# rebots-online/InstantIR

Measured on AMD Instinct MI355X. Metric: denoising steps/sec at 1024x1024 (InstantIR step: previewer UNet + LCM + Aggregator + UNet, CFG), higher is better.
Workload: dtype f16 (fp32 accumulate); 1 GPU; BASELINE configs[1]: 1024x1024, batch 1/GPU, cfg 7.0 (2 rows), 30-step DDIM timetable, preview_start 0, full SDXL+TA-IP UNet x2 + Aggregator per step; images_per_gpu=1, weight_elements=4422072388, graph=True, finite=True, world=1

## Files before the change

instantir_amd/csrc/gemm8.hip:

```cpp
#include "common.h"
#include "gemm_geo.h"
#include "../../include/instantir_hip.h"

namespace {

using iir::Geo;
constexpr int BK = 64;
constexpr int PF_TOUCHES = 2;

template <int BN, bool F8 = false>
__global__ __launch_bounds__(512, 2) void gemm8_kernel(const Geo g) {
    using E = f16;
    using E4 = f16x4;
    using E8 = f16x8;
    constexpr int BM = 256, NT = 512;
    constexpr int WM = 128, WN = BN / 4, MI = WM / 16, NI = WN / 16;
    constexpr int A_BYTES = BM * 128, B_BYTES = BN * 128, STAGE = A_BYTES + B_BYTES, RING_BYTES = 2 * STAGE;
    constexpr int A_PIECES = BM / 64, B_PIECES = BN / 64;
    static_assert(BN % 64 == 0 && NI * 16 == WN && B_PIECES <= MI - 1, "tile shape");
    extern __shared__ __attribute__((aligned(16))) char smem[];
    float2* rowstat = (float2*)(smem + RING_BYTES + 2048);

    const int tid = threadIdx.x, lane = tid & 63;
    const int wave = __builtin_amdgcn_readfirstlane(tid >> 6);
    const int wm = wave >> 2, wn = wave & 3;

    int tm, tn;
    if (!iir::tile_of_block(g, tm, tn)) return;
    const int m0 = tm * BM, n0 = tn * BN;

    const int srow = lane >> 3, schunk = (lane & 7) ^ srow;
    const unsigned a_voff = (unsigned)(srow * (int)g.lda * 2 + schunk * 16);
    const unsigned b_voff = (unsigned)(srow * g.K * 2 + schunk * 16);
    const char* a_base = (const char*)g.A + (long)(m0 + wave * 8) * g.lda * 2;
    const char* b_base = (const char*)g.W + (long)(n0 + wave * 8) * g.K * 2;
    const long a_pstride = 64L * g.lda * 2, b_pstride = 64L * g.K * 2;
    auto stage_a = [&](int t, int buf) {
#pragma unroll
        for (int q = 0; q < A_PIECES; ++q)
            glds16(a_base + q * a_pstride + t * 128 + a_voff, smem + buf * STAGE + (q * 8 + wave) * 1024);
    };
    auto stage_b1 = [&](int t, int buf, int q) {
        glds16(b_base + q * b_pstride + t * 128 + b_voff, smem + buf * STAGE + A_BYTES + (q * 8 + wave) * 1024);
    };

    const int frow = lane & 15, fq = lane >> 4;
    int a_off[2], b_off[2];
#pragma unroll
    for (int s = 0; s < 2; ++s) {
        const int phys = (s * 4 + fq) ^ (frow & 7);
        a_off[s] = (wm * WM + frow) * 128 + phys * 16;
        b_off[s] = A_BYTES + (wn * WN + frow) * 128 + phys * 16;
    }

    f32x4 acc[MI][NI];
#pragma unroll
    for (int i = 0; i < MI; ++i)
#pragma unroll
        for (int j = 0; j < NI; ++j) acc[i][j] = (f32x4){0.f, 0.f, 0.f, 0.f};

    const int nk = g.K / BK;
    stage_a(0, 0);
#pragma unroll
    for (int q = 0; q < B_PIECES; ++q) stage_b1(0, 0, q);
    if (nk > 1) {
#pragma unroll
        for (int q = 0; q < B_PIECES; ++q) stage_b1(1, 1, q);
    }

    if (g.ln_in && tid < BM) rowstat[tid] = iir::ln_row_stat(g, min(m0 + tid, g.M - 1));

    E8 bfr[2][NI], a0[2], a1[2];
    auto read_b = [&](const char* st) {
#pragma unroll
        for (int s = 0; s < 2; ++s)
#pragma unroll
            for (int j = 0; j < NI; ++j) bfr[s][j] = *(const E8*)(st + b_off[s] + j * 2048);
    };
    auto read_a = [&](const char* st, int i, E8 (&a)[2]) {
#pragma unroll
        for (int s = 0; s < 2; ++s) a[s] = *(const E8*)(st + a_off[s] + i * 2048);
    };

    if (nk > 1) asm volatile("s_waitcnt vmcnt(%0)\n\ts_barrier" ::"n"(B_PIECES) : "memory");
    else asm volatile("s_waitcnt vmcnt(0)\n\ts_barrier" ::: "memory");

    int cur = 0;
    for (int t = 0; t < nk; ++t) {
        const char* st = smem + cur * STAGE;
        read_b(st);
        read_a(st, 0, a0);
        const bool more_a = t + 1 < nk, more_b = t + 2 < nk;
        if (more_a) stage_a(t + 1, cur ^ 1);
        auto piece = [&](int i) { if (i >= 1 && i <= B_PIECES && more_b) stage_b1(t + 2, cur, i - 1); };
#pragma unroll
        for (int i = 0; i < MI; ++i) {
            E8(&ac)[2] = (i & 1) ? a1 : a0;
            E8(&an)[2] = (i & 1) ? a0 : a1;
            if (i + 1 < MI) read_a(st, i + 1, an);
            piece(i);
            __builtin_amdgcn_s_setprio(1);
#pragma unroll
            for (int s = 0; s < 2; ++s)
#pragma unroll
                for (int j = 0; j < NI; ++j) {
                    if constexpr (F8) acc[i][j] = iir::mfma16_f8x2(bfr[s][j], ac[s], acc[i][j]);
                    else acc[i][j] = __builtin_amdgcn_mfma_f32_16x16x32_f16(bfr[s][j], ac[s], acc[i][j], 0, 0, 0);
                }
            __builtin_amdgcn_s_setprio(0);
            if (i == 0) asm volatile("s_waitcnt lgkmcnt(0)\n\ts_barrier" ::: "memory");
        }
        if (more_b) asm volatile("s_waitcnt vmcnt(%0) lgkmcnt(0)\n\ts_barrier" ::"n"(B_PIECES) : "memory");
        else asm volatile("s_waitcnt vmcnt(0) lgkmcnt(0)\n\ts_barrier" ::: "memory");
        cur ^= 1;
    }

    const bool paired = g.epi != IIR_EPI_PLAIN;
    const int cs = (paired ? BN : 2 * BN) + 32;
    constexpr int CHUNK_ROWS = 64, STAGE_STRIDE = CHUNK_ROWS * (2 * BN + 32);
    f32x4 c1v[NI], scv[F8 ? NI : 1];
    E4 c0v[NI];
#pragma unroll
    for (int j = 0; j < NI; ++j) {
        const int nc = n0 + wn * WN + j * 16 + fq * 4;
        c1v[j] = g.ln_in ? *(const f32x4*)(g.ln_colsum + nc) : (f32x4){0.f, 0.f, 0.f, 0.f};
        if constexpr (F8) scv[j] = *(const f32x4*)(g.wscale + nc) * g.a_scale;
        if (g.bias) c0v[j] = *(const E4*)(g.bias + nc);
        else for (int t = 0; t < 4; ++t) c0v[j][t] = (E)0.f;
    }
    const int cpr = paired ? BN / 16 : BN / 8;
    const int no_tile = paired ? n0 / 2 : n0;
    const bool use_res = g.res && !paired;
    const int total = CHUNK_ROWS * cpr;
    iir::touch_next_weights<NT, PF_TOUCHES>(g, tid, smem + RING_BYTES + wave * 256);
#pragma unroll
    for (int c = 0; c < MI / 2; ++c) {
        char* ct = smem + (c & 1) * STAGE_STRIDE;
#pragma unroll
        for (int ii = 0; ii < 2; ++ii) {
            const int i = 2 * c + ii;
            const int lr = wm * WM + i * 16 + frow;
            const float2 rs = g.ln_in ? rowstat[lr] : make_float2(1.f, 0.f);
            char* rowp = ct + (wm * 32 + ii * 16 + frow) * cs;
#pragma unroll
            for (int j = 0; j < NI; ++j) {
                float a[4];
#pragma unroll
                for (int t = 0; t < 4; ++t) a[t] = iir::epi_affine(F8 ? acc[i][j][t] * scv[F8 ? j : 0][t] : acc[i][j][t], rs, c1v[j][t], (float)c0v[j][t]);
                if (!paired) {
                    iir::epi_act(g.act, a);
                    E4 o;
                    for (int t = 0; t < 4; ++t) o[t] = (E)a[t];
                    *(E4*)(rowp + (wn * WN + j * 16 + fq * 4) * 2) = o;
                } else {
                    int col;
                    const f16x2 o2 = iir::geglu_pair<E>(a, fq, col);
                    *(f16x2*)(rowp + ((wn * WN + j * 16) / 2 + col) * 2) = o2;
                }
            }
        }
        asm volatile("s_waitcnt lgkmcnt(0)\n\ts_barrier" ::: "memory");
        if (g.Ct && n0 >= g.tr_from) {
#pragma unroll 1
            for (int p = tid; p < BN * (CHUNK_ROWS / 8); p += NT) {
                const int col = p >> 3, gq = p & 7;
                const long m = m0 + (gq >> 2) * WM + c * 32 + (gq & 3) * 8;
                E8 o;
#pragma unroll
                for (int t = 0; t < 8; ++t) o[t] = (E)((float)*(const E*)(ct + (gq * 8 + t) * cs + col * 2) * g.out_scale);
                *(E8*)(g.Ct + (long)(n0 + col - g.tr_from) * g.ldct + m) = o;
            }
            continue;
        }
#pragma unroll 1
        for (int p = tid; p < total; p += NT) {
            const int s = p / cpr, cc = p - s * cpr;
            const long m = m0 + (s >> 5) * WM + c * 32 + (s & 31);
            const E8 v = *(const E8*)(ct + s * cs + cc * 16);
            E8 o;
            if (use_res) {
                const E8 rr = *(const E8*)(g.res + m * g.ldr + no_tile + cc * 8);
                for (int t = 0; t < 8; ++t) o[t] = (E)(((float)v[t] + (float)rr[t]) * g.out_scale);
            } else {
                for (int t = 0; t < 8; ++t) o[t] = (E)((float)v[t] * g.out_scale);
            }
            if (g.c_fp8) *(long*)((char*)g.C + m * g.ldc + no_tile + cc * 8) = iir_fp8x8(o);
            else iir::store16(g.C, (m * g.ldc + no_tile + cc * 8) * 2, o, g.st_wt != 0);
        }
    }
    asm volatile("s_waitcnt vmcnt(0)" ::: "memory");
}

template <int BN, bool F8 = false>
int launch8(const Geo& g0, hipStream_t stream) {
    constexpr int BM = 256;
    Geo g = g0;
    iir::xcd_partition(g, BM, BN, HUGE_VAL);
    const size_t lds = 2 * (BM * 128 + BN * 128) + 2048 + BM * 8;
    static unsigned long long lds_set = 0;
    if (!iir_ensure_dynamic_lds((const void*)gemm8_kernel<BN, F8>, lds, lds_set)) return IIR_ELAUNCH;
    iir_launch(gemm8_kernel<BN, F8>, dim3(8 * g.rm * g.rn), dim3(512), lds, stream, g);
    return iir_launch_status();
}

}

namespace iir {

bool gemm8_covers(const Geo& g, int bn) {
    if (bn != 320 && bn != 256) return false;
    if (g.dtype != IIR_DT_F16 || g.c_f32 || g.ln_out || g.gn_out || (g.wscale && !g.f8) || g.rowbias || g.xa_on) return false;
    if (g.f8 && (g.ln_in || g.Ct || bn != 320)) return false;
    if (g.c_fp8 && (g.ldc % 8 || (uintptr_t)g.C % 8)) return false;
    if (g.Ct && (g.epi != IIR_EPI_PLAIN || g.res || g.tr_from % bn || !g.ct_vec)) return false;
    if (g.epi != IIR_EPI_PLAIN && g.epi != IIR_EPI_GEGLU) return false;
    if (g.M % 256 || g.N % bn || g.K % 64 || g.K < 128) return false;
    if ((!g.c_vec && !g.c_fp8) || (g.res && g.epi == IIR_EPI_PLAIN && !g.r_vec)) return false;
    if (g.lda % 8 || ((uintptr_t)g.A % 16) || ((uintptr_t)g.W % 16)) return false;
    if (g.bias && ((uintptr_t)g.bias % 8)) return false;
    if (g.ln_in && g.ln_parts > 8) return false;
    if ((long)g.lda * 2 * 7 + 128 >= (1L << 31) || (long)g.K * 2 * 7 + 128 >= (1L << 31)) return false;
    return true;
}

int gemm8_launch(const Geo& g, int bn, hipStream_t stream) {
    if (!gemm8_covers(g, bn)) return IIR_EINVAL;
    if (g.f8) return launch8<320, true>(g, stream);
    return bn == 320 ? launch8<320>(g, stream) : launch8<256>(g, stream);
}

}
```

instantir_amd/csrc/gemm_conv.hip:

```cpp
#include "common.h"
#include "gemm_geo.h"
#include "../../include/instantir_hip.h"
#include <stdlib.h>
#include <type_traits>

namespace {

using iir::Geo;

constexpr int BK = 64;
#define IIR_PIN() __builtin_amdgcn_sched_barrier(0)
constexpr int PF_TOUCHES = 4;

constexpr int gn_par(int bm, bool lw) { return lw && bm == 128 ? 2 : 1; }
constexpr int ring_bytes(int bm, int bn, int st, bool w8) { return st * (bm * 128 + (w8 ? bn * 64 : bn * 128)); }
constexpr int scratch_bytes(int waves_m, bool lw) { return 256 * waves_m * 2 * (lw ? 2 : 1); }
constexpr int lds_bytes(int bm, int bn, int st, int waves_m, bool w8, bool lw) { return ring_bytes(bm, bn, st, w8) + scratch_bytes(waves_m, lw) + bm * 8; }
constexpr int lnp_off(int bm, int bn) { return (bm * (2 * bn + 32) + 15) / 16 * 16; }
constexpr bool ln_out_fits(int bm, int bn, int st, bool w8) { return lnp_off(bm, bn) + bm * (bn / 8) * 8 <= ring_bytes(bm, bn, st, w8); }
constexpr bool gn_out_fits(int bm, int bn, int st, int nt, bool lw, bool w8 = false) {
    const int gnt = nt / gn_par(bm, lw);
    return bm % 64 == 0 && bn <= gnt && (long)lnp_off(bm, bn) + (long)gn_par(bm, lw) * (gnt / (bn / 8)) * bn * 8 <= ring_bytes(bm, bn, st, w8);
}

// ... 734 lines not shown
    if (g.gn_out) {
        constexpr bool fits = gn_out_fits(BM, BN, ST, NT, LW, W8);
        if (!fits || g.epi != IIR_EPI_PLAIN || g.c_f32 || g.Ct || g.ln_out || g.M % BM || g.N % BN || !g.c_vec || (g.res && !g.r_vec) ||
            (CONV && (g.y_img_rows | g.res_img_rows)))
            return IIR_EINVAL;
    }
    if (g.ln_out) {
        constexpr bool fits = ln_out_fits(BM, BN, ST, W8);
        if (!fits || CONV || g.epi != IIR_EPI_PLAIN || g.c_f32 || g.Ct || g.M % BM || g.N % BN || !g.c_vec || (g.res && !g.r_vec))
            return IIR_EINVAL;
    }
    iir::xcd_partition(g, BM, BN, 3.0 * 1048576.);
    const dim3 grid(8 * g.rm * g.rn), block(NT);
    const auto kern = gemm_kernel<E, BM, BN, ST, CONV, WAVES_M, W8, LW, F8>;
    static unsigned long long lds_set = 0;
    if (!iir_ensure_dynamic_lds((const void*)kern, lds, lds_set)) return IIR_ELAUNCH;
    iir_launch(kern, grid, block, lds, stream, g);
    return iir_launch_status();
}

template <int BM, int BN, int ST, int WAVES_M = 2, bool LW = false>
int launch(const Geo& g, bool conv, hipStream_t stream) {
    constexpr bool T5_3 = BM == 64 && BN == 160 && ST == 3 && WAVES_M == 2;
    constexpr bool FP8_TILE = T5_3 || (ST == 2 && WAVES_M == 2 && !LW);
    if (g.f8 || g.wscale) {
        if (conv || g.dtype != IIR_DT_F16) return IIR_EINVAL;
        if constexpr (FP8_TILE) {
            if (g.f8) return launch_k<f16, BM, BN, ST, false, WAVES_M, false, LW, true>(g, stream);
            if constexpr (!LW) return launch_k<f16, BM, BN, ST, false, WAVES_M, true>(g, stream);
        }
        return IIR_EINVAL;
    }
    if (g.dtype == IIR_DT_BF16) {
        if constexpr (ST == 2 && WAVES_M == 2 && !LW)
            return conv ? launch_k<bf16, BM, BN, ST, true>(g, stream) : launch_k<bf16, BM, BN, ST, false>(g, stream);
        return IIR_EINVAL;
    }
    if (!conv) return launch_k<f16, BM, BN, ST, false, WAVES_M, false, LW>(g, stream);
    if constexpr (!LW || ST == 3) return launch_k<f16, BM, BN, ST, true, WAVES_M, false, LW>(g, stream);
    return IIR_EINVAL;
}

struct TileShape { int bm, bn; };
constexpr TileShape kTiles[] = {{0, 0}, {128, 128}, {128, 64}, {64, 64}, {128, 160}, {64, 160}, {256, 128}};
constexpr int N_TILES = sizeof(kTiles) / sizeof(kTiles[0]) - 1;

constexpr int ONE_PER_CU_MIN_K = 1280;

int pick_tile(int M, int N, bool paired, int K = 0) {
    if (K >= ONE_PER_CU_MIN_K && (long)((M + 63) / 64) * ((N + 159) / 160) <= 256) return 5;
    long best = -1;
    int pick = 1;
    for (int t = 1; t <= 5; ++t) {
        const long blocks = (long)((M + kTiles[t].bm - 1) / kTiles[t].bm) * ((N + kTiles[t].bn - 1) / kTiles[t].bn);
        const long cost = ((blocks + 511) / 512) * 2 * (kTiles[t].bm + kTiles[t].bn);
        if (best < 0 || cost < best || (cost == best && kTiles[t].bm * kTiles[t].bn > kTiles[pick].bm * kTiles[pick].bn)) {
            best = cost;
            pick = t;
        }
    }
    return pick;
}

struct Resolved { int id, bm, bn, st, nt; bool lw; };

Resolved resolve_tile(int M, int N, int K, bool conv, int dtype, bool wscale, bool f8, int tile) {
    const bool f16 = dtype == IIR_DT_F16;
    if (tile < 0 || tile > N_TILES) return {-1, 0, 0, 0, 0, false};
    if (tile == 0) {
        static const bool t4_lw = !(getenv("IIR_T4_LW") && atoi(getenv("IIR_T4_LW")) == 0);
        if (t4_lw && f16 && !wscale && !f8 && K >= ONE_PER_CU_MIN_K && M % 128 == 0 && N % 160 == 0 &&
            (long)(M / 128) * (N / 160) <= 256 && (long)(M / 64) * (N / 160) > 256 && pick_tile(M, N, false, K) == 5)
            return {54, 128, 160, 3, 512, true};
        tile = pick_tile(M, N, false, K);
    }
    const int bm = kTiles[tile].bm, bn = kTiles[tile].bn;
    const long blocks = (long)((M + bm - 1) / bm) * ((N + bn - 1) / bn);
    const bool one_per_cu = tile == 5 && blocks <= 256 && K >= ONE_PER_CU_MIN_K && f16;
    if (one_per_cu && (!wscale || f8)) return {55, bm, bn, 3, 512, true};
    const int stages = one_per_cu ? 3 : 2;
    return {tile + 10 * stages, bm, bn, stages, tile == 6 ? 512 : 256, false};
}

bool gemm8_auto(const Geo& g, bool conv) {
    return !conv && (g.f8 ? 2 * g.K : g.K) >= 640 && (long)(g.M / 256) * (g.N / 320) >= 256 && iir::gemm8_covers(g, 320);
}

int dispatch(const Geo& g, bool conv, int tile, hipStream_t stream) {
    if (g.xa_on) return conv ? IIR_EINVAL : launch<64, 128, 3>(g, false, stream);
    if (tile == 0 && gemm8_auto(g, conv)) return iir::gemm8_launch(g, 320, stream);
    if (tile == 91 || tile == 92) return conv ? IIR_EINVAL : iir::gemm8_launch(g, tile == 91 ? 320 : 256, stream);
    if (tile < 10) tile = resolve_tile(g.M, g.N, g.f8 ? 2 * g.K : g.K, conv, g.dtype, g.wscale != nullptr, g.f8 != 0, tile).id;
    switch (tile) {
        case 21: return launch<128, 128, 2>(g, conv, stream);
        case 31: return launch<128, 128, 3>(g, conv, stream);
        case 22: return launch<128, 64, 2>(g, conv, stream);
        case 23: return launch<64, 64, 2>(g, conv, stream);
        case 24: return launch<128, 160, 2>(g, conv, stream);
        case 34: return launch<128, 160, 3>(g, conv, stream);
        case 25: return launch<64, 160, 2>(g, conv, stream);
        case 35: return launch<64, 160, 3>(g, conv, stream);
        case 54: return launch<128, 160, 3, 2, true>(g, conv, stream);
        case 55: return launch<64, 160, 3, 2, true>(g, conv, stream);
        case 65: return launch<64, 160, 4, 2, true>(g, conv, stream);
        case 75: return launch<64, 160, 2, 2, true>(g, conv, stream);
        case 26: return launch<256, 128, 2, 4>(g, conv, stream);
        case 36: return launch<256, 128, 3, 4>(g, conv, stream);
        case 90:
            if (g.epi == IIR_EPI_PLAIN) return IIR_EINVAL;
            return launch<256, 320, 2, 4>(g, conv, stream);
        default: return IIR_EINVAL;
    }
}

void finish_geo(Geo& g) {
    g.st_wt = (long)g.M * g.ldc * 2 < (1L << 31);
    if (g.pf_lines <= 0) { g.pf = (const char*)g.W; g.pf_lines = 1; }
    g.c_vec = (g.ldc % 8 == 0) && ((uintptr_t)g.C % 16 == 0);
    g.r_vec = g.res && (g.ldr % 8 == 0) && ((uintptr_t)g.res % 16 == 0);
}

}

extern "C" int iir_gemm_tile_bn(int32_t tile) { tile %= 10; return (tile >= 1 && tile <= N_TILES) ? kTiles[tile].bn : -1; }

extern "C" int iir_gemm_pick_tile(int32_t M, int32_t N, int32_t K, int32_t paired) { return pick_tile(M, N, paired != 0, K); }

extern "C" int iir_gemm_ln_parts(int32_t M, int32_t N, int32_t K) {
    if (M <= 0 || N <= 0 || K <= 0) return 0;
    const Resolved r = resolve_tile(M, N, K, false, IIR_DT_F16, false, false, 0);
    if (M % r.bm || N % r.bn || N / r.bn > 8) return 0;
    return N / r.bn;
}

static int fill_gemm_geo(const iir_gemm_desc* d, Geo& g);

extern "C" int iir_gemm_gn_supported(int32_t M, int32_t N, int32_t K, int32_t is_conv) {
    if (M <= 0 || N <= 0 || K <= 0 || M % 64) return 0;
    const Resolved r = resolve_tile(M, N, K, is_conv != 0, IIR_DT_F16, false, false, 0);
    if (M % r.bm || N % r.bn) return 0;
    return gn_out_fits(r.bm, r.bn, r.st, r.nt, r.lw) ? 1 : 0;
}

extern "C" int iir_gemm_fp8_out_supported(int32_t M, int32_t N, int32_t K, int32_t paired) {
    if (M <= 0 || N <= 0 || K <= 0 || K % 128) return 0;
    (void)paired;
    const Resolved r = resolve_tile(M, N, K, false, IIR_DT_F16, true, true, 0);
    return (M % r.bm == 0 && N % r.bn == 0) ? 1 : 0;
}

extern "C" int iir_gemm_f16(const iir_gemm_desc* d, void* stream) {
    (void)hipGetLastError();
    Geo g{};
    const int rc = fill_gemm_geo(d, g);
    if (rc != IIR_OK) return rc;
    return dispatch(g, false, d->tile, (hipStream_t)stream);
}

extern "C" int iir_gemm_resolve_tile(const iir_gemm_desc* d) {
    Geo g{};
    if (fill_gemm_geo(d, g) != IIR_OK) return -1;
    if (g.xa_on) return 93;
    if (d->tile != 0) return d->tile;
    if (gemm8_auto(g, false)) return 91;
    return resolve_tile(g.M, g.N, g.f8 ? 2 * g.K : g.K, false, g.dtype, g.wscale != nullptr, g.f8 != 0, 0).id;
}

static int fill_gemm_geo(const iir_gemm_desc* d, Geo& g) {
    if (!d || !d->A || !d->W || !d->C) return IIR_EINVAL;
    if (d->M <= 0 || d->N <= 0 || d->K <= 0 || d->K % BK) return IIR_EINVAL;
    if (d->N % 4 || d->lda % 8 || d->ldc % 4) return IIR_EINVAL;
    if (d->epi != IIR_EPI_PLAIN && (d->N % 16)) return IIR_EINVAL;
    if (d->epi == IIR_EPI_SFT && !d->res) return IIR_EINVAL;
    if (d->rowbias && d->rows_per_rb <= 0) return IIR_EINVAL;
    if (d->epi < IIR_EPI_PLAIN || d->epi > IIR_EPI_XATTN) return IIR_EINVAL;
    if (d->epi == IIR_EPI_XATTN) {
        const iir_attn_kv* kv = d->xattn_kv;
        if (!kv || d->dtype != IIR_DT_F16 || d->N % 128 || d->M % 64 || d->xattn_tq <= 0 || d->xattn_tq % 64 || d->M % d->xattn_tq) return IIR_EINVAL;
        if (d->res || d->rowbias || d->act || d->Ct || d->c_f32 || d->wscale || d->ln_stats_out || d->gn_stats_out) return IIR_EINVAL;
        if (d->ldc % 8 || (uintptr_t)d->C % 16 || (d->tile != 0 && d->tile != 93)) return IIR_EINVAL;
        if (kv[0].Tkv < 1 || kv[0].Tkv > 80 || kv[1].Tkv < 1 || kv[1].Tkv > 64) return IIR_EINVAL;
        for (int sgm = 0; sgm < 2; ++sgm) {
            if (!kv[sgm].K || !kv[sgm].Vt || (uintptr_t)kv[sgm].K % 16 || (uintptr_t)kv[sgm].Vt % 16) return IIR_EINVAL;
            if (kv[sgm].ldk % 8 || kv[sgm].k_batch_stride % 8 || kv[sgm].ldvt % 8 || kv[sgm].vt_batch_stride % 8) return IIR_EINVAL;
            g.xa_k[sgm] = (const f16*)kv[sgm].K; g.xa_ldk[sgm] = kv[sgm].ldk; g.xa_kb[sgm] = kv[sgm].k_batch_stride;
            g.xa_vt[sgm] = (const f16*)kv[sgm].Vt; g.xa_ldvt[sgm] = kv[sgm].ldvt; g.xa_vb[sgm] = kv[sgm].vt_batch_stride;
            g.xa_tk[sgm] = kv[sgm].Tkv;
        }
        g.xa_on = 1; g.xa_tq = d->xattn_tq;
    }
    g.A = (const f16*)d->A; g.lda = d->lda; g.W = (const f16*)d->W; g.C = (f16*)d->C; g.ldc = d->ldc;
    g.M = d->M; g.N = d->N; g.K = d->K;
    g.bias = (const f16*)d->bias; g.rowbias = (const f16*)d->rowbias; g.ldrb = d->ldrb; g.rows_per_rb = d->rows_per_rb;
    g.res = (const f16*)d->res; g.ldr = d->ldr; g.epi = d->epi == IIR_EPI_XATTN ? IIR_EPI_PLAIN : d->epi; g.act = d->act;
    g.out_scale = d->out_scale == 0.f ? 1.f : d->out_scale;
    g.pf = (const char*)d->prefetch; g.pf_lines = d->prefetch ? (int)(d->prefetch_bytes / 128) : 0;
    finish_geo(g);
    if (d->dtype != IIR_DT_F16 && d->dtype != IIR_DT_BF16) return IIR_EINVAL;
    g.dtype = d->dtype;
    if (d->c_f32) {
        if (d->epi != IIR_EPI_PLAIN || d->bias || d->rowbias || d->res || d->Ct || d->act || d->ldc % 4 || (uintptr_t)d->C % 16) return IIR_EINVAL;
        g.c_f32 = 1;
    }
    if (d->wscale) {
        if (d->c_f32 || d->K % 64 || (uintptr_t)d->W % 16 || (uintptr_t)d->wscale % 16 || d->dtype != IIR_DT_F16) return IIR_EINVAL;
        g.wscale = (const float*)d->wscale;
    }
    if (d->c_fp8) {
        if (d->epi == IIR_EPI_XATTN || d->epi == IIR_EPI_SFT || d->c_f32 || d->Ct || d->ln_stats_out || d->gn_stats_out || d->dtype != IIR_DT_F16) return IIR_EINVAL;
        g.c_fp8 = 1;
    }
    g.a_scale = 1.f;
    if (d->a_fp8) {
        if (!d->wscale || d->K % 128 || d->lda % 16 || (uintptr_t)d->A % 16 || d->ln_stats_in || d->epi == IIR_EPI_XATTN) return IIR_EINVAL;
        g.f8 = 1;
        g.a_scale = d->a_scale == 0.f ? 1.f : d->a_scale;
        g.K = d->K / 2; g.lda = d->lda / 2;
    }
    if (d->Ct) {
        if (d->epi != IIR_EPI_PLAIN || d->tr_from < 0 || d->tr_from >= d->N || d->tr_from % 8 || d->ldct < d->M) return IIR_EINVAL;
        g.Ct = (f16*)d->Ct; g.ldct = d->ldct; g.tr_from = d->tr_from;
        g.ct_vec = (d->ldct % 8 == 0) && ((uintptr_t)d->Ct % 16 == 0);
    }
    if (d->ln_stats_out) {
        if ((uintptr_t)d->ln_stats_out % 8 || d->c_f32 || d->Ct || d->epi != IIR_EPI_PLAIN) return IIR_EINVAL;
        g.ln_out = (float*)d->ln_stats_out;
    }
    if (d->gn_stats_out) {
        if ((uintptr_t)d->gn_stats_out % 8 || d->M % 64 || d->epi != IIR_EPI_PLAIN || d->c_f32 || d->Ct || d->ln_stats_out || d->wscale) return IIR_EINVAL;
        g.gn_out = (float*)d->gn_stats_out;
    }
    if (d->ln_stats_in) {
        if (!d->ln_colsum || d->ln_parts <= 0 || d->ln_parts > 8 || d->ln_part_cols <= 0 || (long)d->ln_parts * d->ln_part_cols != d->K || d->c_f32 ||
            (uintptr_t)d->ln_stats_in % 8 || (uintptr_t)d->ln_colsum % 16 || !(d->ln_eps > 0.f)) return IIR_EINVAL;
        g.ln_in = (const float*)d->ln_stats_in; g.ln_colsum = (const float*)d->ln_colsum;
        g.ln_parts = d->ln_parts; g.ln_part_cols = d->ln_part_cols; g.ln_eps = d->ln_eps;
    }
    return IIR_OK;
}

extern "C" int iir_conv2d_nhwc_f16(const iir_conv_desc* c, void* stream) {
    (void)hipGetLastError();
    if (!c || !c->X || !c->Wt || !c->Y || !c->zero_page) return IIR_EINVAL;
    if (c->ksize != 3 && c->ksize != 1) return IIR_EINVAL;
    if (c->Cin % BK || c->ldx % 8 || c->Cout % 4 || c->ldy % 4) return IIR_EINVAL;
    if (c->stride != 1 && c->stride != 2) return IIR_EINVAL;
    if (c->upsample && c->stride != 1) return IIR_EINVAL;
// ... 29 lines not shown
```

instantir_amd/csrc/gemm_geo.h:

```cpp
#pragma once
#include "common.h"
#include "../../include/instantir_hip.h"
#include <math.h>

namespace iir {

typedef unsigned iir_u32x4 __attribute__((ext_vector_type(4)));
template <typename V>
__device__ __forceinline__ void store16(void* base, long byte_off, const V& v, bool wt) {
    static_assert(sizeof(V) == 16, "16-byte chunk");
    if (wt) {
        __amdgpu_buffer_rsrc_t r = __builtin_amdgcn_make_buffer_rsrc(base, 0, 0x7FFFFFFF, 0x00020000);
        __builtin_amdgcn_raw_buffer_store_b128(__builtin_bit_cast(iir_u32x4, v), r, (int)byte_off, 0, 16);
    } else {
        *(V*)((char*)base + byte_off) = v;
    }
}

struct Geo {
    const f16* A; long lda;
    const f16* W;
    f16* C; long ldc;
    int M, N, K;
    const f16* bias;
// ... 4 lines not shown
    int H, Wd, Cin, Ho, Wo, ks, stride, pad, ups;
    const f16* zero;
    long x_img_stride;
    int y_img_rows, res_img_rows;
    int tiles_m, tiles_n;
    int xm, rm, rn;
    const char* pf; int pf_lines;
    f16* Ct; long ldct; int tr_from, ct_vec;
    int c_vec, r_vec;
    int dtype;
    int c_f32;
    const float* wscale;
    float* ln_out;
    const float* ln_in;
    int ln_parts, ln_part_cols;
    float ln_eps;
    float* gn_out;
    int st_wt;
    const float* ln_colsum;
    int xa_on, xa_tq;
    const f16* xa_k[2]; long xa_ldk[2], xa_kb[2];
    const f16* xa_vt[2]; long xa_ldvt[2], xa_vb[2];
    int xa_tk[2];
    int c_fp8;
    int f8; float a_scale;
};


__device__ __forceinline__ bool tile_of_block(const Geo& g, int& tm, int& tn) {
    const int bid = (int)blockIdx.x, xcd = bid & 7, local = bid >> 3;
    const int rx = xcd % g.xm, ry = xcd / g.xm;
    tm = rx * g.rm + local % g.rm;
    tn = ry * g.rn + local / g.rm;
    return tm < g.tiles_m && tn < g.tiles_n;
}

static inline void xcd_partition(Geo& g, int bm, int bn, double a_keep_bytes) {
    g.tiles_m = (g.M + bm - 1) / bm;
    g.tiles_n = (g.N + bn - 1) / bn;
    double best = -1.;
    const double row_bytes = (double)g.K * 2.;
    for (int xm = 1; xm <= 8; xm *= 2) {
        const int xn = 8 / xm;
        const int rm = (g.tiles_m + xm - 1) / xm, rn = (g.tiles_n + xn - 1) / xn;
        const double a_bytes = (double)rm * bm * row_bytes, w_bytes = (double)rn * bn * row_bytes;
        const int cols_per_group = rm >= 64 ? 1 : 64 / rm;
        const double groups = (double)((rn + cols_per_group - 1) / cols_per_group);
        double cost = (a_bytes <= a_keep_bytes ? a_bytes : a_bytes * groups) + w_bytes;
        cost += ((double)rm * rn * 8 - (double)g.tiles_m * g.tiles_n) * 8. * 64 * (bm + bn);
        if (best < 0. || cost < best) { best = cost; g.xm = xm; g.rm = rm; g.rn = rn; }
    }
}

__device__ __forceinline__ float2 ln_row_stat(const Geo& g, int m) {
    constexpr int MAXP = 8;
    float2 lnp_in[MAXP];
#pragma unroll
    for (int j = 0; j < MAXP; ++j) lnp_in[j] = ((const float2*)g.ln_in)[(long)min(j, g.ln_parts - 1) * g.M + m];
    float sm = 0.f;
#pragma unroll
    for (int j = 0; j < MAXP; ++j) sm += j < g.ln_parts ? lnp_in[j].x : 0.f;
    const float inv_p = 1.0f / (float)g.ln_parts, mean = sm * inv_p;
    float m2 = 0.f, dev = 0.f;
#pragma unroll
    for (int j = 0; j < MAXP; ++j) {
        const float d = lnp_in[j].x - mean;
        m2 += j < g.ln_parts ? lnp_in[j].y : 0.f;
        dev += j < g.ln_parts ? d * d : 0.f;
    }
    const float var = (m2 + (float)g.ln_part_cols * dev) * inv_p / (float)g.ln_part_cols;
    const float rstd = rsqrtf(var + g.ln_eps);
    return make_float2(rstd, -rstd * mean);
}

template <typename V>
__device__ __forceinline__ f32x4 mfma16_f8x2(V w, V a, f32x4 c) {
    typedef long l2 __attribute__((ext_vector_type(2)));
    const l2 w2 = __builtin_bit_cast(l2, w), a2 = __builtin_bit_cast(l2, a);
    c = __builtin_amdgcn_mfma_f32_16x16x32_fp8_fp8(w2[0], a2[0], c, 0, 0, 0);
    return __builtin_amdgcn_mfma_f32_16x16x32_fp8_fp8(w2[1], a2[1], c, 0, 0, 0);
}

__device__ __forceinline__ float epi_affine(float x, float2 rs, float colsum, float bias) { return fmaf(x, rs.x, fmaf(rs.y, colsum, bias)); }
__device__ __forceinline__ void epi_act(int act, float (&v)[4]) {
    if (act == IIR_ACT_SILU) for (int t = 0; t < 4; ++t) v[t] = silu_f(v[t]);
    else if (act == IIR_ACT_GELU) for (int t = 0; t < 4; ++t) v[t] = gelu_erf_f(v[t]);
    else if (act == IIR_ACT_QUICKGELU) for (int t = 0; t < 4; ++t) v[t] = quick_gelu_f(v[t]);
}

template <typename E>
__device__ __forceinline__ auto geglu_pair(const float (&a)[4], int fq, int& col) {
    typedef E E2 __attribute__((ext_vector_type(2)));
    float b[4];
#pragma unroll
    for (int t = 0; t < 4; ++t) b[t] = __shfl_xor(a[t], 32, 64);
    const bool gate = fq >= 2;
    col = (fq & 1) * 4 + (gate ? 2 : 0);
    const float v0 = gate ? b[2] : a[0], v1 = gate ? b[3] : a[1], g0 = gate ? a[2] : b[0], g1 = gate ? a[3] : b[1];
    return (E2){(E)(v0 * gelu_erf_f(g0)), (E)(v1 * gelu_erf_f(g1))};
}

template <int NT, int TOUCHES>
__device__ __forceinline__ void touch_next_weights(const Geo& g, int tid, char* scratch) {
    const int per = (g.pf_lines + (int)gridDim.x - 1) / (int)gridDim.x;
    const long l0 = (long)blockIdx.x * per, last = g.pf_lines - 1;
#pragma unroll
    for (int i = 0; i < TOUCHES; ++i) {
        long l = l0 + min(tid + i * NT, per - 1);
        if (l > last) l = last;
        __builtin_amdgcn_global_load_lds((const GLOBAL_AS void*)(g.pf + l * 128), (LDS_AS void*)scratch, 4, 0, 0);
    }
}

int gemm8_launch(const Geo& g, int bn, hipStream_t stream);
bool gemm8_covers(const Geo& g, int bn);

}
```

instantir_amd/ops.py:

```python
from __future__ import annotations

import ctypes as C

import torch

from . import lib as L
from .lib import ACT_GELU, ACT_NONE, ACT_QUICKGELU, ACT_SILU, EPI_GEGLU, EPI_PLAIN, EPI_SFT, EPI_XATTN


def _stream():
    return torch.cuda.current_stream().cuda_stream


def _p(t):
    return None if t is None else t.data_ptr()


_DT = {torch.float16: 0, torch.bfloat16: 1}


def _chk2d(t, name, dtype=torch.float16):
    if t.dtype != dtype or t.dim() != 2 or t.stride(1) != 1 or not t.is_cuda:
        raise ValueError(f"{name}: expected a 2-D {dtype} CUDA tensor with unit column stride, got {t.dtype} {tuple(t.shape)} {t.stride()}")

# ... 204 lines not shown
        raise ValueError(msg)
    d.Ct, d.ldct, d.tr_from = ct.data_ptr(), ct.stride(0), tr_from


def _fill_kv(table, kv):
    for i, (k, k_rows, vt, vbs, tkv) in enumerate(kv):
        _chk2d(k, "k"); _chk2d(vt, "vt")
        e = table[i]
        e.K, e.ldk, e.k_batch_stride = k.data_ptr(), k.stride(0), k_rows * k.stride(0)
        e.Vt, e.ldvt, e.vt_batch_stride = vt.data_ptr(), vt.stride(0), vbs
        e.Tkv = tkv


def gemm(a, w, out, bias=None, rowbias=None, rows_per_rb=1, res=None, epi=EPI_PLAIN, act=ACT_NONE, out_scale=1.0,
         tile=0, prefetch=None, out_t=None, wscale=None, ln_out=None, ln_in=None, gn_out=None, xattn=None):
    dt = a.dtype
    if isinstance(w, Fp8Weight):
        w, wscale = w.q, w.scale
    if wscale is not None:
        if w.dtype not in (torch.float8_e4m3fn, torch.uint8) or w.dim() != 2 or not w.is_contiguous() or not w.is_cuda:
            raise ValueError("fp8 weights: contiguous 2-D CUDA tensor of torch.float8_e4m3fn (or its bytes)")
        if wscale.dtype != torch.float32 or wscale.numel() != w.shape[0] or not wscale.is_contiguous():
            raise ValueError("wscale: contiguous fp32 (N,)")
        if dt != torch.float16:
            raise ValueError("fp8 weights take fp16 activations")
    if dt not in _DT:
        raise ValueError(f"a: fp16 or bf16 expected, got {dt}")
    c_f32 = out.dtype == torch.float32
    _chk2d(a, "a", dt); _chk2d(out, "out", torch.float32 if c_f32 else dt)
    if wscale is None:
        _chk2d(w, "w", dt)
    for t_, n_ in ((bias, "bias"), (rowbias, "rowbias"), (res, "res")):
        if t_ is not None and t_.dtype != dt:
            raise ValueError(f"{n_}: dtype {t_.dtype} does not match the operands ({dt})")
    M, K = a.shape
    N = w.shape[0]
    if w.shape[1] != K or not w.is_contiguous():
        raise ValueError("w must be contiguous (N,K) with K matching a")
    n_out = (N if epi in (EPI_PLAIN, EPI_XATTN) else N // 2) if out_t is None else out_t[1]
    if out.shape != (M, n_out):
        raise ValueError(f"out shape {tuple(out.shape)} != {(M, n_out)}")
    d = L.GemmDesc()
    d.A, d.lda = a.data_ptr(), a.stride(0)
    d.W = w.data_ptr()
    d.C, d.ldc = out.data_ptr(), out.stride(0)
    d.M, d.N, d.K = M, N, K
    d.bias = _p(bias)
    _fill_operands(d, dt, M, N, rowbias, rows_per_rb, res, prefetch, gn_out)
    d.epi, d.act, d.out_scale, d.tile = epi, act, out_scale, tile
    d.dtype, d.c_f32 = _DT[dt], int(c_f32)
    if wscale is not None:
        d.wscale = wscale.data_ptr()
    if ln_out is not None:
        if ln_out.dtype != torch.float32 or not ln_out.is_contiguous() or ln_out.dim() != 3 or ln_out.shape[1:] != (M, 2) \
                or ln_out.shape[0] != ln_parts(M, N, K) or tile != 0:
            raise ValueError("ln_out: contiguous fp32 (ln_parts(M, N, K), M, 2), tile = 0")
        d.ln_stats_out = ln_out.data_ptr()
    if ln_in is not None:
        part, colsum, eps = ln_in
        if part.dtype != torch.float32 or not part.is_contiguous() or part.dim() != 3 or part.shape[1:] != (M, 2) or K % part.shape[0]:
            raise ValueError("ln_in partials: contiguous fp32 (parts, M, 2) with parts dividing K")
        if colsum.dtype != torch.float32 or colsum.numel() != N or not colsum.is_contiguous():
            raise ValueError("ln_in colsum: contiguous fp32 (N,)")
        d.ln_stats_in, d.ln_colsum, d.ln_parts, d.ln_part_cols, d.ln_eps = part.data_ptr(), colsum.data_ptr(), part.shape[0], K // part.shape[0], eps
    kv_keep = None
    if (epi == EPI_XATTN) != (xattn is not None):
        raise ValueError("epi = EPI_XATTN goes with xattn = (kv, Tq)")
    if xattn is not None:
        kvs, tq = xattn
        if len(kvs) != 2:
            raise ValueError("xattn: two K / V^T segments (text, IP tokens)")
        kv_keep = (L.AttnKV * 2)()
        _fill_kv(kv_keep, kvs)
        d.xattn_kv, d.xattn_tq = kv_keep, tq
    if xattn is not None:
        tile = 93
    elif tile == 0:
        tile = auto_tile(M, N, epi != EPI_PLAIN, K)
    if out_t is not None:
        _fill_out_t(d, out_t, dt, M, N, False, "out_t must hold (N - tr_from, M)")
    No = N // 2 if epi not in (EPI_PLAIN, EPI_XATTN) else N
    if xattn is not None:
        cls = "gemm_kernel<64x128,gemm+xattn>"
    elif PROFILER is not None and d.tile == 0 and L.load().iir_gemm_resolve_tile(C.byref(d)) == 91:
        cls = "gemm8_kernel<256x320,gemm>"
    else:
        cls = "gemm_kernel<%s,%s>" % (_TILE_NAMES[tile % 10], "gemm" if wscale is None else "gemm-w8")
    xa_flops = 4.0 * M * N * sum(k[4] for k in xattn[0]) if xattn is not None else 0.0
    with _Timed(cls, 2.0 * M * N * K + xa_flops,
                2.0 * (M * K + N * K * (1.0 if wscale is None else 0.5) + M * No + (M * No if res is not None else 0))):
        L.check(L.load().iir_gemm_f16(C.byref(d), _stream()), "iir_gemm_f16")
    return out


def conv2d(x, w, out, ksize=3, stride=1, upsample=False, bias=None, rowbias=None, rows_per_rb=1, res=None,
           epi=EPI_PLAIN, act=ACT_NONE, out_scale=1.0, tile=0, y_img_rows=0, res_img_rows=0, pad_mode=0, prefetch=None, gn_out=None):
    R, H, Wd, Cin = x.shape
    dt = x.dtype
    if dt not in _DT or x.stride(3) != 1 or x.stride(1) != Wd * x.stride(2):
        raise ValueError("x must be an NHWC fp16 / bf16 view with dense rows (pixel and image strides are free)")
    _chk2d(out, "out", dt)
    for t_, n_ in ((w, "w"), (bias, "bias"), (rowbias, "rowbias"), (res, "res")):
        if t_ is not None and t_.dtype != dt:
            raise ValueError(f"{n_}: dtype {t_.dtype} does not match x ({dt})")
    Cout = w.shape[0]
    if tuple(w.shape[1:]) != (ksize, ksize, Cin) or not w.is_contiguous():
        raise ValueError("w must be contiguous (Cout,k,k,Cin)")
    d = L.ConvDesc()
    d.X, d.ldx = x.data_ptr(), x.stride(2)
    d.R, d.H, d.Wd, d.Cin = R, H, Wd, Cin
    d.Wt = w.data_ptr()
    d.Y, d.ldy = out.data_ptr(), out.stride(0)
    d.Cout, d.ksize, d.stride, d.upsample = Cout, ksize, stride, int(bool(upsample))
    d.bias = _p(bias)
    d.dtype = _DT[dt]
    Hi, Wi = (2 * H, 2 * Wd) if upsample else (H, Wd)
    pad2 = 1 if pad_mode == 1 else 2 * (ksize // 2)
    Mo = R * ((Hi + pad2 - ksize) // stride + 1) * ((Wi + pad2 - ksize) // stride + 1)
    _fill_operands(d, dt, Mo, Cout, rowbias, rows_per_rb, res, prefetch, gn_out)
    d.epi, d.act, d.out_scale, d.tile = epi, act, out_scale, tile
    if tile == 0:
        Kc = ksize * ksize * Cin
        tile = auto_tile(Mo, Cout, epi != EPI_PLAIN, Kc)
    d.zero_page = zero_page(x.device).data_ptr()
    d.x_img_stride, d.y_img_rows, d.res_img_rows, d.pad_mode = x.stride(0), y_img_rows, res_img_rows, pad_mode
    Co = Cout // 2 if epi != EPI_PLAIN else Cout
    with _Timed("gemm_kernel<%s,conv>" % _TILE_NAMES[tile % 10], 2.0 * Mo * Cout * ksize * ksize * Cin,
                2.0 * (R * H * Wd * Cin + Cout * ksize * ksize * Cin + Mo * Co + (Mo * Co if res is not None else 0))):
        L.check(L.load().iir_conv2d_nhwc_f16(C.byref(d), _stream()), "iir_conv2d_nhwc_f16")
    return out


ATTN_LOG2E = 1.4426950408889634


def attn_q_factor(scale=0.125):
    import numpy as np
    return float(np.float32(scale) * np.float32(ATTN_LOG2E))


def attention(q, o, kv, batch, heads, Tq, scale=0.125, causal=False, q_prescaled=False, head_dim=64, ident_from=0):
    _chk2d(q, "q")
    d = L.AttnDesc()
    if o.dtype in _FP8_DTYPES:
        if o.dim() != 2 or o.stride(1) != 1 or o.stride(0) % 4 or not o.is_cuda:
            raise ValueError("attention: an fp8 `o` needs contiguous rows with a stride % 4 == 0")
        d.o_fp8 = 1
    else:
        _chk2d(o, "o")
    d.Q, d.ldq, d.q_batch_stride = q.data_ptr(), q.stride(0), Tq * q.stride(0)
    d.O, d.ldo, d.o_batch_stride = o.data_ptr(), o.stride(0), Tq * o.stride(0)
    d.batch, d.heads, d.Tq, d.nseg, d.scale = batch, heads, Tq, len(kv), scale
    d.causal = int(bool(causal))
    d.q_prescaled = int(bool(q_prescaled))
    _fill_kv(d.kv, kv)
    if ident_from:
        if head_dim != 64:
            raise ValueError("attention: identity rows need head_dim 64")
        with _Timed("attn_kernel", 4.0 * ident_from * heads * Tq * head_dim * kv[0][4],
                    2.0 * ident_from * heads * head_dim * (2 * Tq + 2 * kv[0][4]) + 4.0 * (batch - ident_from) * heads * Tq * head_dim):
            L.check(L.load().iir_attention_d64_ident_f16(C.byref(d), int(ident_from), _stream()), "iir_attention_d64_ident_f16")
        return o
    with _Timed("attn_kernel", 4.0 * batch * heads * Tq * head_dim * sum(k[4] for k in kv),
                2.0 * batch * heads * head_dim * (2 * Tq + 2 * sum(k[4] for k in kv))):
        if head_dim == 64:
            L.check(L.load().iir_attention_d64_f16(C.byref(d), _stream()), "iir_attention_d64_f16")
        else:
            L.check(L.load().iir_attention_f16(C.byref(d), head_dim, _stream()), "iir_attention_f16")
# ... 462 lines not shown
```

Baseline: 17.41 steps/s.

## Specialize gemm8 epilogue at compile time and auto-route transposed-output GEMMs to 256-wide tile

Templates the gemm8 kernel on whether the epilogue is GEGLU and dispatches on the activation with compile-time tags. This removes runtime branches and makes the staging stride constant. The GEGLU cross-half exchange now uses permlane32 swaps instead of shuffles, and the row-stat array is always filled so the epilogue loses a branch. Separately, the auto-dispatch now sends transposed-output GEMMs with large K and roughly one wave of 256x256 tiles to the 256-wide gemm8 variant. This adds template instantiations and can change which kernel runs for some shapes.

Result: faster. 17.80 steps/s (median of 6 runs) (+2.3%).

```diff
diff --git a/instantir_amd/csrc/gemm8.hip b/instantir_amd/csrc/gemm8.hip
--- a/instantir_amd/csrc/gemm8.hip
+++ b/instantir_amd/csrc/gemm8.hip
@@ -1,5 +1,6 @@
 #include "common.h"
 #include "gemm_geo.h"
+#include <type_traits>
 #include "../../include/instantir_hip.h"
 
 namespace {
@@ -8,7 +9,7 @@
 constexpr int BK = 64;
 constexpr int PF_TOUCHES = 2;
 
-template <int BN, bool F8 = false>
+template <int BN, bool F8, bool GEGLU>
 __global__ __launch_bounds__(512, 2) void gemm8_kernel(const Geo g) {
     using E = f16;
     using E4 = f16x4;
@@ -68,7 +69,7 @@
         for (int q = 0; q < B_PIECES; ++q) stage_b1(1, 1, q);
     }
 
-    if (g.ln_in && tid < BM) rowstat[tid] = iir::ln_row_stat(g, min(m0 + tid, g.M - 1));
+    if (tid < BM) rowstat[tid] = g.ln_in ? iir::ln_row_stat(g, min(m0 + tid, g.M - 1)) : make_float2(1.f, 0.f);
 
     E8 bfr[2][NI], a0[2], a1[2];
     auto read_b = [&](const char* st) {
@@ -115,8 +116,7 @@
         cur ^= 1;
     }
 
-    const bool paired = g.epi != IIR_EPI_PLAIN;
-    const int cs = (paired ? BN : 2 * BN) + 32;
+    constexpr int cs = (GEGLU ? BN : 2 * BN) + 32;
     constexpr int CHUNK_ROWS = 64, STAGE_STRIDE = CHUNK_ROWS * (2 * BN + 32);
     f32x4 c1v[NI], scv[F8 ? NI : 1];
     E4 c0v[NI];
@@ -128,39 +128,48 @@
         if (g.bias) c0v[j] = *(const E4*)(g.bias + nc);
         else for (int t = 0; t < 4; ++t) c0v[j][t] = (E)0.f;
     }
-    const int cpr = paired ? BN / 16 : BN / 8;
-    const int no_tile = paired ? n0 / 2 : n0;
-    const bool use_res = g.res && !paired;
-    const int total = CHUNK_ROWS * cpr;
+    constexpr int cpr = GEGLU ? BN / 16 : BN / 8;
+    const int no_tile = GEGLU ? n0 / 2 : n0;
+    const bool use_res = g.res && !GEGLU;
+    constexpr int total = CHUNK_ROWS * cpr;
+    const int pair_col = iir::geglu_col(fq);
     iir::touch_next_weights<NT, PF_TOUCHES>(g, tid, smem + RING_BYTES + wave * 256);
-#pragma unroll
-    for (int c = 0; c < MI / 2; ++c) {
-        char* ct = smem + (c & 1) * STAGE_STRIDE;
+    auto phase1 = [&](int c, char* ct, auto act_tag) {
+        constexpr int ACT = decltype(act_tag)::value;
 #pragma unroll
         for (int ii = 0; ii < 2; ++ii) {
             const int i = 2 * c + ii;
             const int lr = wm * WM + i * 16 + frow;
-            const float2 rs = g.ln_in ? rowstat[lr] : make_float2(1.f, 0.f);
+            const float2 rs = rowstat[lr];
             char* rowp = ct + (wm * 32 + ii * 16 + frow) * cs;
 #pragma unroll
             for (int j = 0; j < NI; ++j) {
                 float a[4];
 #pragma unroll
                 for (int t = 0; t < 4; ++t) a[t] = iir::epi_affine(F8 ? acc[i][j][t] * scv[F8 ? j : 0][t] : acc[i][j][t], rs, c1v[j][t], (float)c0v[j][t]);
-                if (!paired) {
-                    iir::epi_act(g.act, a);
+                if constexpr (!GEGLU) {
+                    iir::epi_act<ACT>(a);
                     E4 o;
-                    for (int t = 0; t < 4; ++t) o[t] = (E)a[t];
+                    for (int t = 0; t < 4; ++t) o[t] = (E)iir::rounded_f32(a[t]);
                     *(E4*)(rowp + (wn * WN + j * 16 + fq * 4) * 2) = o;
                 } else {
-                    int col;
-                    const f16x2 o2 = iir::geglu_pair<E>(a, fq, col);
-                    *(f16x2*)(rowp + ((wn * WN + j * 16) / 2 + col) * 2) = o2;
+                    *(f16x2*)(rowp + ((wn * WN + j * 16) / 2 + pair_col) * 2) = iir::geglu_pair<E>(a);
                 }
             }
         }
+    };
+#pragma unroll
+    for (int c = 0; c < MI / 2; ++c) {
+        char* ct = smem + (c & 1) * STAGE_STRIDE;
+        if constexpr (GEGLU) phase1(c, ct, std::integral_constant<int, IIR_ACT_NONE>{});
+        else switch (g.act) {
+            case IIR_ACT_SILU: phase1(c, ct, std::integral_constant<int, IIR_ACT_SILU>{}); break;
+            case IIR_ACT_GELU: phase1(c, ct, std::integral_constant<int, IIR_ACT_GELU>{}); break;
+            case IIR_ACT_QUICKGELU: phase1(c, ct, std::integral_constant<int, IIR_ACT_QUICKGELU>{}); break;
+            default: phase1(c, ct, std::integral_constant<int, IIR_ACT_NONE>{}); break;
+        }
         asm volatile("s_waitcnt lgkmcnt(0)\n\ts_barrier" ::: "memory");
-        if (g.Ct && n0 >= g.tr_from) {
+        if (!GEGLU && g.Ct && n0 >= g.tr_from) {
 #pragma unroll 1
             for (int p = tid; p < BN * (CHUNK_ROWS / 8); p += NT) {
                 const int col = p >> 3, gq = p & 7;
@@ -191,16 +200,21 @@
     asm volatile("s_waitcnt vmcnt(0)" ::: "memory");
 }
 
+template <int BN, bool F8, bool GEGLU>
+int launch8_form(const Geo& g, hipStream_t stream) {
+    constexpr int BM = 256;
+    const size_t lds = 2 * (BM * 128 + BN * 128) + 2048 + BM * 8;
+    static unsigned long long lds_set = 0;
+    if (!iir_ensure_dynamic_lds((const void*)gemm8_kernel<BN, F8, GEGLU>, lds, lds_set)) return IIR_ELAUNCH;
+    iir_launch(gemm8_kernel<BN, F8, GEGLU>, dim3(8 * g.rm * g.rn), dim3(512), lds, stream, g);
+    return iir_launch_status();
+}
+
 template <int BN, bool F8 = false>
 int launch8(const Geo& g0, hipStream_t stream) {
-    constexpr int BM = 256;
     Geo g = g0;
-    iir::xcd_partition(g, BM, BN, HUGE_VAL);
-    const size_t lds = 2 * (BM * 128 + BN * 128) + 2048 + BM * 8;
-    static unsigned long long lds_set = 0;
-    if (!iir_ensure_dynamic_lds((const void*)gemm8_kernel<BN, F8>, lds, lds_set)) return IIR_ELAUNCH;
-    iir_launch(gemm8_kernel<BN, F8>, dim3(8 * g.rm * g.rn), dim3(512), lds, stream, g);
-    return iir_launch_status();
+    iir::xcd_partition(g, 256, BN, HUGE_VAL);
+    return g.epi == IIR_EPI_GEGLU ? launch8_form<BN, F8, true>(g, stream) : launch8_form<BN, F8, false>(g, stream);
 }
 
 }
diff --git a/instantir_amd/csrc/gemm_conv.hip b/instantir_amd/csrc/gemm_conv.hip
--- a/instantir_amd/csrc/gemm_conv.hip
+++ b/instantir_amd/csrc/gemm_conv.hip
@@ -840,13 +840,23 @@
     return {tile + 10 * stages, bm, bn, stages, tile == 6 ? 512 : 256, false};
 }
 
-bool gemm8_auto(const Geo& g, bool conv) {
-    return !conv && (g.f8 ? 2 * g.K : g.K) >= 640 && (long)(g.M / 256) * (g.N / 320) >= 256 && iir::gemm8_covers(g, 320);
+int gemm8_auto(const Geo& g, bool conv) {
+    if (conv) return 0;
+    const int K = g.f8 ? 2 * g.K : g.K;
+    if (K >= 640 && (long)(g.M / 256) * (g.N / 320) >= 256 && iir::gemm8_covers(g, 320)) return 320;
+    if (g.Ct && K >= 1280 && g.N % 256 == 0 && iir::gemm8_covers(g, 256)) {
+        const long tiles = (long)(g.M / 256) * (g.N / 256);
+        if (tiles >= 240 && tiles <= 256) return 256;
+    }
+    return 0;
 }
 
 int dispatch(const Geo& g, bool conv, int tile, hipStream_t stream) {
     if (g.xa_on) return conv ? IIR_EINVAL : launch<64, 128, 3>(g, false, stream);
-    if (tile == 0 && gemm8_auto(g, conv)) return iir::gemm8_launch(g, 320, stream);
+    if (tile == 0) {
+        const int bn8 = gemm8_auto(g, conv);
+        if (bn8) return iir::gemm8_launch(g, bn8, stream);
+    }
     if (tile == 91 || tile == 92) return conv ? IIR_EINVAL : iir::gemm8_launch(g, tile == 91 ? 320 : 256, stream);
     if (tile < 10) tile = resolve_tile(g.M, g.N, g.f8 ? 2 * g.K : g.K, conv, g.dtype, g.wscale != nullptr, g.f8 != 0, tile).id;
     switch (tile) {
@@ -920,7 +930,8 @@
     if (fill_gemm_geo(d, g) != IIR_OK) return -1;
     if (g.xa_on) return 93;
     if (d->tile != 0) return d->tile;
-    if (gemm8_auto(g, false)) return 91;
+    const int bn8 = gemm8_auto(g, false);
+    if (bn8) return bn8 == 320 ? 91 : 92;
     return resolve_tile(g.M, g.N, g.f8 ? 2 * g.K : g.K, false, g.dtype, g.wscale != nullptr, g.f8 != 0, 0).id;
 }
 
diff --git a/instantir_amd/csrc/gemm_geo.h b/instantir_amd/csrc/gemm_geo.h
--- a/instantir_amd/csrc/gemm_geo.h
+++ b/instantir_amd/csrc/gemm_geo.h
@@ -110,22 +110,32 @@
 }
 
 __device__ __forceinline__ float epi_affine(float x, float2 rs, float colsum, float bias) { return fmaf(x, rs.x, fmaf(rs.y, colsum, bias)); }
-__device__ __forceinline__ void epi_act(int act, float (&v)[4]) {
-    if (act == IIR_ACT_SILU) for (int t = 0; t < 4; ++t) v[t] = silu_f(v[t]);
-    else if (act == IIR_ACT_GELU) for (int t = 0; t < 4; ++t) v[t] = gelu_erf_f(v[t]);
-    else if (act == IIR_ACT_QUICKGELU) for (int t = 0; t < 4; ++t) v[t] = quick_gelu_f(v[t]);
+__device__ __forceinline__ float rounded_f32(float x) {
+    asm("" : "+v"(x));
+    return x;
 }
 
+template <int ACT>
+__device__ __forceinline__ void epi_act(float (&v)[4]) {
+    if constexpr (ACT == IIR_ACT_SILU) for (int t = 0; t < 4; ++t) v[t] = silu_f(v[t]);
+    else if constexpr (ACT == IIR_ACT_GELU) for (int t = 0; t < 4; ++t) v[t] = gelu_erf_f(v[t]);
+    else if constexpr (ACT == IIR_ACT_QUICKGELU) for (int t = 0; t < 4; ++t) v[t] = quick_gelu_f(v[t]);
+}
+
+__device__ __forceinline__ void xhalf_swap(float lo, float hi, float& first, float& second) {
+    const auto s = __builtin_amdgcn_permlane32_swap(__float_as_uint(lo), __float_as_uint(hi), false, false);
+    first = __uint_as_float(s[0]);
+    second = __uint_as_float(s[1]);
+}
+
+__device__ __forceinline__ int geglu_col(int fq) { return (fq & 1) * 4 + (fq >= 2 ? 2 : 0); }
 template <typename E>
-__device__ __forceinline__ auto geglu_pair(const float (&a)[4], int fq, int& col) {
+__device__ __forceinline__ auto geglu_pair(const float (&a)[4]) {
     typedef E E2 __attribute__((ext_vector_type(2)));
-    float b[4];
-#pragma unroll
-    for (int t = 0; t < 4; ++t) b[t] = __shfl_xor(a[t], 32, 64);
-    const bool gate = fq >= 2;
-    col = (fq & 1) * 4 + (gate ? 2 : 0);
-    const float v0 = gate ? b[2] : a[0], v1 = gate ? b[3] : a[1], g0 = gate ? a[2] : b[0], g1 = gate ? a[3] : b[1];
-    return (E2){(E)(v0 * gelu_erf_f(g0)), (E)(v1 * gelu_erf_f(g1))};
+    float v0, g0, v1, g1;
+    xhalf_swap(a[0], a[2], v0, g0);
+    xhalf_swap(a[1], a[3], v1, g1);
+    return (E2){(E)rounded_f32(v0 * gelu_erf_f(g0)), (E)rounded_f32(v1 * gelu_erf_f(g1))};
 }
 
 template <int NT, int TOUCHES>
diff --git a/instantir_amd/ops.py b/instantir_amd/ops.py
--- a/instantir_amd/ops.py
+++ b/instantir_amd/ops.py
@@ -310,8 +310,8 @@
     No = N // 2 if epi not in (EPI_PLAIN, EPI_XATTN) else N
     if xattn is not None:
         cls = "gemm_kernel<64x128,gemm+xattn>"
-    elif PROFILER is not None and d.tile == 0 and L.load().iir_gemm_resolve_tile(C.byref(d)) == 91:
-        cls = "gemm8_kernel<256x320,gemm>"
+    elif PROFILER is not None and d.tile == 0 and L.load().iir_gemm_resolve_tile(C.byref(d)) in (91, 92):
+        cls = "gemm8_kernel<256x%d,gemm>" % (320 if L.load().iir_gemm_resolve_tile(C.byref(d)) == 91 else 256)
     else:
         cls = "gemm_kernel<%s,%s>" % (_TILE_NAMES[tile % 10], "gemm" if wscale is None else "gemm-w8")
     xa_flops = 4.0 * M * N * sum(k[4] for k in xattn[0]) if xattn is not None else 0.0
```
